# ranrandy/gaussian-splatting-mpm

Hardware: AMD Instinct MI355X
Metric: MPM substeps/sec (and particles·steps/sec) + rendered fps, lego 128³ grid (higher is better)
Workload: dtype f32; 1 GPU; lego.json frame: 100 substeps + postprocess + render 800x800 SH3; particles_per_gpu=100000, particles_total=100000, n_grid=128, material=jelly, render_overlap=True, render_first=False, render_thread=True, render_async=False, parallelism=single

## Files before the change

### gaussian-splatting-mpm_amd/csrc/fused.h

```cpp

#ifndef GSMPM_FT2
#define GSMPM_FT2 7
#endif
constexpr int kFT0 = 8, kFT1 = 8, kFT2 = GSMPM_FT2;
constexpr int kFW0 = kFT0 + 4, kFW1 = kFT1 + 4, kFW2 = kFT2 + 4;
constexpr int kFWin = kFW0 * kFW1 * kFW2;
constexpr int kFTN = kFT0 * kFT1 * kFT2;

__device__ __forceinline__ int slot_loc(int w0, int w1, int w2) { return (w0 * kFW1 + w1) * kFW2 + w2; }

struct SlabWin {
  int W;
  int a[2];
  int on[2];
  float4* part[2];
  int y0[2], ny[2];
  int z0[2], nz[2];
  int* oob;
  int pass;
};

__device__ __forceinline__ int slab_window_of(const SlabWin& sw, int i) {
  if (sw.on[0] && i >= sw.a[0] && i < sw.a[0] + sw.W) return 0;
  if (sw.on[1] && i >= sw.a[1] && i < sw.a[1] + sw.W) return 1;
// ... 15 lines not shown
  int td0, td1, td2;
  int ntiles;
  int max_chunks;
};

struct BinOutF {
  int* count;
  int* ptile;
  int* pslot;
  int* tflag;
  FTiles tl;
};

struct FusedRare {
  BinOutF bo;
  float4* gacc;
  int* esc;
  int* drift;
  int* nonfin;
  const void* bct;
  int* tflag;
  int* touched;
  int* nchunk;
  int4* chunk;
  int2* rcov;
  int* tbox;
  const int* tpos;
  int* rbox;
  const float4* slots_prev;
  const int* tbox_prev;
  const float4* gacc_prev;
  const int* esc_prev;
  const int* esc_old;
  float4* gacc_old;
  int* esc_clr;
  float grav[3];
  unsigned* esc_count;
  float4* esc_nodes;
  unsigned* vmax;
};

constexpr int kFT[3] = {kFT0, kFT1, kFT2};
#ifndef GSMPM_FOLD_BATCH
#define GSMPM_FOLD_BATCH 1
#endif
constexpr int kFoldB = GSMPM_FOLD_BATCH;
__device__ __forceinline__ void fold_axis(int w, int T, int& d, int& sec) {
// ... 136 lines not shown
  tc[0] = b[0] / kFT0;
  tc[1] = b[1] / kFT1;
  tc[2] = b[2] / kFT2;
  return ok ? (tc[0] * tl.td1 + tc[1]) * tl.td2 + tc[2] : tl.ntiles;
}

__device__ __noinline__ void mark8(int* __restrict__ tflag, int t, int td0, int td1, int td2) {
  const int tz = t % td2, ty = (t / td2) % td1, tx = t / (td1 * td2);
  for (int a = 0; a <= 1; ++a)
    for (int b = 0; b <= 1; ++b)
      for (int c = 0; c <= 1; ++c)
        if (tx + a < td0 && ty + b < td1 && tz + c < td2) tflag[((tx + a) * td1 + ty + b) * td2 + tz + c] = 1;
}
__device__ __forceinline__ int reserve_f(const BinOutF& bo, int t, int c) {
  const int old = atomicAdd(&bo.count[t], c);
  if (old == 0 && t < bo.tl.ntiles) mark8(bo.tflag, t, bo.tl.td0, bo.tl.td1, bo.tl.td2);
  return old;
}

struct Touch {
  int* tflag;
  int* touched;
  int* nchunk;
  int4* chunk;
  int* cbox;
  int* tbox;
  unsigned char* perm;
  int2* rcov;
  const int* tpos;
  int* rbox;
};

__device__ __forceinline__ int balanced_lane(const int* __restrict__ rcnt, int cnt, int r, int rank) {
  const int Lr = (cnt - r + 15) >> 4;
  if (rank < Lr) return rank * 16 + r;
  int o = rank - Lr;
  for (int q = 0; q < r; ++q) o += max(0, rcnt[q] - ((cnt - q + 15) >> 4));
  int acc = 0;
  for (int q = 0; q < 16; ++q) {
    const int Lq = (cnt - q + 15) >> 4, d = max(0, Lq - rcnt[q]);
    if (o < acc + d) return (rcnt[q] + (o - acc)) * 16 + q;
    acc += d;
  }
  return rank * 16 + r;
}

constexpr int kFullBox = 0 | (0 << 4) | (0 << 8) | ((kFW0 - 1) << 12) | ((kFW1 - 1) << 16) | ((kFW2 - 1) << 20);
__device__ __forceinline__ void box_unpack(int b, int (&lo)[3], int (&hi)[3]) {
// ... 385 lines not shown
```

### gaussian-splatting-mpm_amd/csrc/fused_body.inc

```
#ifndef GSMPM_FUSED_BODY_INCLUDER
#error "fused_body.inc is the body of k_fused / k_fused_mixed: it is included inside those two kernels in fused.h only"
#endif
  constexpr bool G2P = (MODE & 1) != 0, P2G = (MODE & 2) != 0;
  constexpr bool FOLD = G2P && (MODE & 4) != 0;
  __shared__ int s_fc0[27], s_fnc[27], s_fbx[27];
  constexpr int kEscMax = kFWin / 27;
  __shared__ int s_nesc;
  __shared__ int s_eb[3][kEscMax];
  GridStep fgs{};
  bool fesc = false;
  if constexpr (FOLD) {
    fgs.dt = dt;
    fgs.dgx = dt * rare->grav[0];
    fgs.dgy = dt * rare->grav[1];
    fgs.dgz = dt * rare->grav[2];
    fgs.mask = mask_prev;
    fgs.keep = 0;
    fesc = __builtin_amdgcn_readfirstlane(*rare->esc_prev) != 0;
  }
  __shared__ unsigned long long s_acc[4 * kFWin];
  __shared__ float s_max[4];
  __shared__ int s_mxy[4], s_mz[4];
  __shared__ int s_cnt[27], s_base[27];
  __shared__ int s_rcnt[16];
  float4* s_win = reinterpret_cast<float4*>(s_acc);
  const int ng = g.ng;
  constexpr int SK = (MODE & 3) == 3 ? 0 : 1;
  sim_prio();
  stamp(SK, 0);
  const int w0 = min((int)blockIdx.x, tl.max_chunks - 1);
  const bool perm0 = use_box && tc.perm;
  const int* nch_p = ck.nchunk;
  const int4* chk_p = ck.chunk;
  const int* cbx_p = tc.cbox;
  const unsigned char* prm_p = perm0 ? tc.perm : reinterpret_cast<const unsigned char*>(tc.cbox);
  asm volatile("" : "+s"(nch_p), "+s"(chk_p), "+s"(cbx_p), "+s"(prm_p));
  typedef const int __attribute__((address_space(1)))* gint_p;
  typedef const unsigned char __attribute__((address_space(1)))* guc_p;
  const gint_p c4 = (gint_p)chk_p + 4 * (size_t)w0;
  const int r0 = c4[0], r1 = c4[1], r2 = c4[2], r3 = c4[3];
  const int bx0 = ((gint_p)cbx_p)[w0];
  const int qv0 = ((guc_p)prm_p)[perm0 ? (size_t)w0 * 256 + threadIdx.x : 0];
  const int nch = *(gint_p)nch_p;
  int4 cr_n = make_int4(r0, r1, r2, r3);
  int box_n = use_box ? bx0 : kFullBox;
  int q_n = perm0 ? qv0 : (int)threadIdx.x;
  for (int w = blockIdx.x; w < nch; w += gridDim.x) {
    const int4 cr = cr_n;
    const int cbox = box_n, q_lane = q_n;
    if (w + (int)gridDim.x < nch) {
      const int wn = w + gridDim.x;
      cr_n = ck.chunk[wn];
      box_n = use_box ? tc.cbox[wn] : kFullBox;
      q_n = (use_box && tc.perm) ? (int)tc.perm[(size_t)wn * 256 + threadIdx.x] : (int)threadIdx.x;
    }
    const int t = cr.x, first = cr.y, cnt = cr.z;
    const int k = threadIdx.x;
    const bool outside = t == tl.ntiles;
    int tx = 0, ty = 0, tz = 0;
    if (!outside) ftile_decode(tl, t, tx, ty, tz);
    const int o0 = tx * kFT0 - 1, o1 = ty * kFT1 - 1, o2 = tz * kFT2 - 1;
    int tpos_e = -1;
    const int* __restrict__ tposp = rare->tpos;
    if (tposp && !outside && k < 27) {
      const int x0 = tx - (k / 9 - 1), y0 = ty - ((k / 3) % 3 - 1), z0 = tz - (k % 3 - 1);
      if ((unsigned)x0 < (unsigned)tl.td0 && (unsigned)y0 < (unsigned)tl.td1 && (unsigned)z0 < (unsigned)tl.td2)
        tpos_e = tposp[(x0 * tl.td1 + y0) * tl.td2 + z0];
    }
    int p = -1;
    float x[3] = {0.f, 0.f, 0.f}, v[3] = {0.f, 0.f, 0.f}, C[3][3], F[3][3], m = 0.f;
    const int q = k >= cnt ? k : q_lane;
    if (k < cnt) {
      p = first + q;
#pragma unroll
      for (int d = 0; d < 3; ++d) x[d] = ps.ld(PX + d, p);
      if (G2P || MAT != 0) {
#pragma unroll
        for (int i = 0; i < 9; ++i) F[i / 3][i % 3] = ps.ld(PF + i, p);
      }
      if (P2G) m = ps.ld(PMASS, p);
      if (!G2P) {
#pragma unroll
        for (int d = 0; d < 3; ++d) v[d] = ps.ld(PV + d, p);
#pragma unroll
        for (int i = 0; i < 9; ++i) C[i / 3][i % 3] = ps.ld(PC + i, p);
      }
    }
    int eslot = -1;
    if constexpr (G2P) {
      if (FOLD && !outside) {
        if (k < 27) {
          const int x0 = tx + k / 9 - 1, y0 = ty + (k / 3) % 3 - 1, z0 = tz + k % 3 - 1;
          int c0 = 0, nc = 0, bx = 0;
          if ((unsigned)x0 < (unsigned)tl.td0 && (unsigned)y0 < (unsigned)tl.td1 && (unsigned)z0 < (unsigned)tl.td2) {
            const int u = (x0 * tl.td1 + y0) * tl.td2 + z0;
            c0 = ck.cbase[u];
            nc = (ck.count[u] + kChunk - 1) / kChunk;
            bx = rare->tbox_prev[u];
          }
          s_fc0[k] = c0;
          s_fnc[k] = nc;
          s_fbx[k] = bx;
        }
        if (k == 0) s_nesc = 0;
        __syncthreads();
        if (k < cnt) {
          int bq[3];
          base_of(x, g.inv_dx, bq);
          if (!(in_grid(x, g) && in_window(bq, o0, o1, o2))) {
// ... 37 lines not shown
          }
          float4 vv[kFoldB][8];
#pragma unroll
          for (int u = 0; u < kFoldB; ++u) fold_load(sp, fn[u], vv[u]);
#pragma unroll
          for (int u = 0; u < kFoldB; ++u) {
            const int ix = o0 + w3[u][0], iy = o1 + w3[u][1], iz = o2 + w3[u][2];
            float4 val = make_float4(0.f, 0.f, 0.f, 0.f);
            if (gin[u]) {
              float4 sum = fold_acc(sp, w3[u], tab, fn[u], vv[u]);
              if (fesc) add4f(sum, rare->gacc_prev[((size_t)ix * ng + iy) * ng + iz]);
              val = node_update(sum, ix, iy, iz, g, fgs, fbct);
            }
            if (live[u]) s_win[(w3[u][0] * kFW1 + w3[u][1]) * kFW2 + w3[u][2]] = val;
          }
        }
        __syncthreads();
        const int ne = min(s_nesc, kEscMax);
        for (int t = k; t < ne * 27; t += 256) {
          const int sl = t / 27, qn = t - sl * 27;
          s_win[kFWin + t] = fold_node(s_eb[0][sl] + qn / 9, s_eb[1][sl] + (qn / 3) % 3, s_eb[2][sl] + qn % 3, g, tl,
                                       ck, rare, fgs, fbct, fesc);
        }
      } else if (!outside) {
        int lo[3], hi[3];
        box_unpack(cbox, lo, hi);
        const int n1 = hi[1] - lo[1] + 1, n2 = hi[2] - lo[2] + 1, n12 = n1 * n2;
        const int nvol = (hi[0] - lo[0] + 1) * n12;
        const float r12 = 1.0f / (float)n12, r2 = 1.0f / (float)n2;
        constexpr int kStageU = (kFWin + 255) / 256;
        float4 gv[kStageU];
        int dst[kStageU];
        bool gin[kStageU];
#pragma unroll
        for (int u = 0; u < kStageU; ++u) {
          const int qn = min(k + u * 256, nvol - 1);
          const int a = (int)(((float)qn + 0.5f) * r12), rem = qn - a * n12;
          const int b = (int)(((float)rem + 0.5f) * r2), c = rem - b * n2;
          const int wa = lo[0] + a, wb = lo[1] + b, wc = lo[2] + c;
          dst[u] = (wa * kFW1 + wb) * kFW2 + wc;
          const int ix = o0 + wa, iy = o1 + wb, iz = o2 + wc;
          gin[u] = (unsigned)ix < (unsigned)ng && (unsigned)iy < (unsigned)ng && (unsigned)iz < (unsigned)ng;
          gv[u] = gvel[gin[u] ? ((size_t)ix * ng + iy) * ng + iz : 0];
        }
#pragma unroll
        for (int u = 0; u < kStageU; ++u) {
          const float4 z = gv[u];
          const bool in = gin[u];
          const float4 val = make_float4(in ? z.x : 0.f, in ? z.y : 0.f, in ? z.z : 0.f, in ? z.w : 0.f);
          if (k + u * 256 < nvol) s_win[dst[u]] = val;
        }
      }
      if (k < 27) s_cnt[k] = 0;
      __syncthreads();
      if (w == (int)blockIdx.x) {
        stamp(SK, 2);
        stamp_val(SK, 5, cnt);
        stamp_val(SK, 6, GSMPM_HWREG(4));
        stamp_val(SK, 7, GSMPM_HWREG(20));
      }
      int code = -1, lslot = 0, nt = -1;
      if (k < cnt) {
        int b[3];
        base_of(x, g.inv_dx, b);
        float gvd[3][3];
        const bool inwin = !outside && in_grid(x, g) && in_window(b, o0, o1, o2);
        const bool eslds = eslot >= 0 && eslot < kEscMax;
        if (FOLD && !inwin && !eslds) {
          float4* en = rare->esc_nodes + (size_t)p * 27;
#pragma unroll 1
          for (int qn = 0; qn < 27; ++qn)
            en[qn] = fold_node(b[0] + qn / 9, b[1] + (qn / 3) % 3, b[2] + qn % 3, g, tl, ck, rare, fgs,
                               static_cast<const BcTable*>(rare->bct), fesc);
// ... 167 lines not shown
        for (int r = 0; r < 3; ++r) {
          vm = fmaxf(vm, fabsf(v[r]));
#pragma unroll
          for (int c = 0; c < 3; ++c) {
            cm = fmaxf(cm, fabsf(C[r][c]));
            sm = fmaxf(sm, fabsf(nvt[r][c]));
          }
        }
        bound = fmaxf(m, m * (vm + 4.5f * g.dx * cm) + dt * 4.5f * g.inv_dx * sm) * 1.01f;
      }
      if (outside) {
        if (k < cnt) {
          p2g_global<MAT>(x, v, C, m, nvt, g, dt, rare->gacc);
          int bq[3];
          base_of(x, g.inv_dx, bq);
          mark_escape_tiles(rare->tflag, rare->touched, rare->nchunk + 1, rare->rcov, tl, ng, bq[0], bq[1], bq[2]);
        }
        if (k == 0 && cnt > 0) {
          *rare->esc = 1;
          atomicAdd(rare->esc_count, (unsigned)cnt);
        }
        if (tc.perm && k < cnt) tc.perm[(size_t)w * 256 + k] = (unsigned char)q;
        __syncthreads();
        continue;
      }
      int b[3];
      base_of(x, g.inv_dx, b);
      const bool win = k < cnt && in_grid(x, g) && in_window(b, o0, o1, o2);
      if (k < cnt && (b[0] < xlo || b[0] >= xhi)) *rare->drift = 1;
      int mxy = win ? (7 << (b[0] - o0)) | (7 << (16 + b[1] - o1)) : 0;
      int mz = win ? 7 << (b[2] - o2) : 0;
      if constexpr (GSMPM_DPP_REDUCE != 0) {
        bound = wave_max_nonneg_dpp(bound);
        mxy = wave_or_dpp(mxy);
        mz = wave_or_dpp(mz);
      } else {
#pragma unroll
        for (int o = 32; o > 0; o >>= 1) {
          bound = fmaxf(bound, __shfl_xor(bound, o));
          mxy |= __shfl_xor(mxy, o);
          mz |= __shfl_xor(mz, o);
        }
      }
      if ((k & 63) == 0) {
        s_max[k >> 6] = bound;
        s_mxy[k >> 6] = mxy;
        s_mz[k >> 6] = mz;
      }
      __syncthreads();
      const int res = win ? (((b[0] - o0) * kFW1 + (b[1] - o1)) * kFW2 + (b[2] - o2)) & 15 : (q & 15);
      const int rrank = (tc.perm && k < cnt) ? atomicAdd(&s_rcnt[res], 1) : 0;
      const float bmax = fmaxf(fmaxf(s_max[0], s_max[1]), fmaxf(s_max[2], s_max[3]));
      const int Mxy = s_mxy[0] | s_mxy[1] | s_mxy[2] | s_mxy[3], Mz = s_mz[0] | s_mz[1] | s_mz[2] | s_mz[3];
      const int Mx = Mxy & 0xffff, My = (unsigned)Mxy >> 16;
      const int lo_all = (Mx & 1) | ((My & 1) << 1) | ((Mz & 1) << 2);
      if (lo_all & ~cr.w) {
        Touch tr = tc;
        tr.tflag = rare->tflag;
        tr.touched = rare->touched;
        tr.nchunk = rare->nchunk;
        tr.rcov = rare->rcov;
        add_lower_tiles(tr, tl, tx, ty, tz, (lo_all | cr.w) & 7);
        if (k == 0) rare->chunk[w].w = lo_all | cr.w;
      }
      int box = kFullBox;
      if (Mx && My && Mz)
        box = (__builtin_ctz(Mx)) | (__builtin_ctz(My) << 4) | (__builtin_ctz(Mz) << 8) | ((31 - __builtin_clz(Mx)) << 12) |
              ((31 - __builtin_clz(My)) << 16) | ((31 - __builtin_clz(Mz)) << 20);
      else
        box = 0;
      if (k == 0) {
        tc.cbox[w] = box;
        rare->tbox[t] = (cr.w & 8) ? kFullBox : box;
      }
      if (tpos_e >= 0) rare->rbox[(size_t)tpos_e * kRecStride + k] = (cr.w & 8) ? kFullBox : box;
      if (cr.w & 8) box = kFullBox;
      int ebits;
      frexpf(bmax, &ebits);
      const int S = bmax > 0.f ? 50 - ebits : 0;
      if (k < cnt) {
        if (win) {
          int bb[3];
          float fx[3], ww[3][3], dw[3][3];
          bspline(x, g.inv_dx, bb, fx, ww, dw);
          p2g_scatter<MAT, kFW1, kFW2, kFWin>(s_acc + ((b[0] - o0) * kFW1 + (b[1] - o1)) * kFW2 + (b[2] - o2), fx, ww,
                                              dw, v, C, m, nvt, g, dt, ldexp(1.0, S));
        } else {
          p2g_global<MAT>(x, v, C, m, nvt, g, dt, rare->gacc);
          *rare->esc = 1;
        }
      }
      {
        const unsigned long long eb = __ballot(k < cnt && !win);
        if (eb) {
          if ((k & 63) == 0) atomicAdd(rare->esc_count, (unsigned)__popcll(eb));
// ... 4 lines not shown
      __syncthreads();
      if (w == (int)blockIdx.x) stamp(SK, 4);
      if (tc.perm && k < cnt) tc.perm[(size_t)w * 256 + balanced_lane(s_rcnt, cnt, res, rrank)] = (unsigned char)q;
      int lo[3], hi[3];
      box_unpack(box, lo, hi);
      const int n1 = hi[1] - lo[1] + 1, n2 = hi[2] - lo[2] + 1, n12 = n1 * n2;
      const int nvol = (hi[0] - lo[0] + 1) * n12;
      const float r12 = 1.0f / (float)n12, r2 = 1.0f / (float)n2;
      const int cid = (cr.w & 16) ? (int)((unsigned)cr.w >> 5) : w;
      float4* dst = slots + (size_t)cid * kFWin;
      for (int qn = k; qn < nvol; qn += 256) {
        const int a = (int)(((float)qn + 0.5f) * r12), rem = qn - a * n12;
        const int bq = (int)(((float)rem + 0.5f) * r2), c = rem - bq * n2;
        const int node = ((lo[0] + a) * kFW1 + lo[1] + bq) * kFW2 + lo[2] + c;
        float4 r;
        r.x = from_fixed32(s_acc[0 * kFWin + node], S);
        r.y = from_fixed32(s_acc[1 * kFWin + node], S);
        r.z = from_fixed32(s_acc[2 * kFWin + node], S);
        r.w = from_fixed32(s_acc[3 * kFWin + node], S);
        wt_store4(dst + node, r);
      }
      __syncthreads();
    }
  }
  if (bin == 2) {
    const BinOutF bo = rare->bo;
    for (int t = blockIdx.x * 256 + threadIdx.x; t <= tl.ntiles; t += gridDim.x * 256) {
      bo.count[t] = 0;
      if (t < tl.ntiles) bo.tflag[t] = 0;
    }
  }
  if (rare->esc_clr) {
    if (__builtin_amdgcn_readfirstlane(*rare->esc_old) != 0) {
      const size_t nn = (size_t)ng * ng * ng;
      for (size_t q = (size_t)blockIdx.x * 256 + threadIdx.x; q < nn; q += (size_t)gridDim.x * 256)
        rare->gacc_old[q] = make_float4(0.f, 0.f, 0.f, 0.f);
    }
    if (blockIdx.x == 0 && threadIdx.x == 0) *rare->esc_clr = 0;
  }
  stamp(SK, 1);
```

### gaussian-splatting-mpm_amd/csrc/mpm.hip

```cpp
#include <hip/hip_runtime.h>
#include <dlfcn.h>


#include <algorithm>
#include <climits>
#include <cmath>
#include <cstring>
#include <map>
#include <numeric>
#include <vector>

#include "common.h"
#include "constitutive.h"
#include <hip/hip_ext.h>

#include "mpm_common.h"
#include "svd3.h"

namespace gsmpm {

#ifndef GSMPM_REBIN_SF
#define GSMPM_REBIN_SF 20
#endif
constexpr int kRebinStressFree = GSMPM_REBIN_SF;
// ... 777 lines not shown
    if (w == (int)blockIdx.x) stamp(1, 4);
    if (p >= 0) {
      bo.ptile[p] = nt;
      bo.pslot[p] = code >= 0 ? s_base[code] + lslot : reserve(bo, nt, 1);
    }
    __syncthreads();
  }
  stamp(1, 1);
}

__global__ __launch_bounds__(256) void k_bin_all(Particles ps, GridDims g, Tiles tl, BinOut bo) {
  const int p = blockIdx.x * blockDim.x + threadIdx.x;
  if (p < ps.n) {
    float x[3];
#pragma unroll
    for (int d = 0; d < 3; ++d) x[d] = ps.ld(PX + d, p);
    int tc[3];
    const int t = tile_of(x, g, tl, tc);
    bo.ptile[p] = t;
    bo.pslot[p] = reserve(bo, t, 1);
  }
}

struct ChunkOut {
  int* cstart;
  int* cbase;
  int4* chunk;
  int* nchunk;
  const int* tflag;
  int* touched;
  int2* rcov = nullptr;
  int* tpos = nullptr;
  int td1 = 0, td2 = 0;
};

constexpr int kRecStride = 32;
__device__ __forceinline__ void write_cover_record(const ChunkOut& co, int ntiles, int E, int t, int rk,
                                                   const int* s_off, const int* s_aux, int total) {
  const int td12 = co.td1 * co.td2, td0 = ntiles / td12;
  const int tz = t % co.td2, ty = (t / co.td2) % co.td1, tx = t / td12;
  for (int e = 0; e < 27; ++e) {
    const int x = tx + e / 9 - 1, y = ty + (e / 3) % 3 - 1, z = tz + e % 3 - 1;
    int2 r = make_int2(0, 0);
    if ((unsigned)x < (unsigned)td0 && (unsigned)y < (unsigned)co.td1 && (unsigned)z < (unsigned)co.td2) {
      const int u = (x * co.td1 + y) * co.td2 + z;
      const int cnt = (u + 1 < E ? s_off[u + 1] : total) - s_off[u];
      r = make_int2(s_aux[u] & 0xffff, (cnt + kChunk - 1) / kChunk);
    }
    co.rcov[(size_t)rk * kRecStride + e] = r;
  }
  co.rcov[(size_t)rk * kRecStride + 27] = make_int2(0, 0);
}

__device__ __forceinline__ int wave_incl_scan(int v) {
  const int lane = threadIdx.x & 63;
#pragma unroll
// ... 69 lines not shown
  for (int t = t0; t < t1; ++t) {
    const int e = s_off[t], c = e & INT_MAX;
    v[0] += c;
    v[1] += (c + kChunk - 1) / kChunk;
    v[2] += e < 0;
  }
  int o[3], tot[3];
  block_scan3(v, o, tot);
  stamp(2, 3);
  for (int t = t0; t < t1; ++t) {
    const int e = s_off[t], c = e & INT_MAX;
    s_off[t] = o[0];
    s_aux[t] = o[1] | (o[2] << 16);
    o[0] += c;
    o[1] += (c + kChunk - 1) / kChunk;
    o[2] += e < 0;
  }
  if (blockIdx.x == 0 && threadIdx.x == 0) {
    co.nchunk[0] = tot[1];
    co.nchunk[1] = tot[2];
  }
  __syncthreads();
  stamp(2, 4);
  const int R = (E + gridDim.x - 1) / gridDim.x;
  for (int t = blockIdx.x * R + threadIdx.x; t < min(E, (int)(blockIdx.x + 1) * R); t += 256) {
    const int off = s_off[t], aux = s_aux[t];
    const int c = (t + 1 < E ? s_off[t + 1] : tot[0]) - off;
    const int cb = aux & 0xffff, rk = aux >> 16;
    const bool touched = (t + 1 < E ? (s_aux[t + 1] >> 16) : tot[2]) > rk;
    co.cbase[t] = cb;
    for (int k = 0; k * kChunk < c; ++k)
      co.chunk[cb + k] = make_int4(t, off + k * kChunk, min(kChunk, c - k * kChunk), c > kChunk ? 8 : 0);
    if (touched) co.touched[rk] = t;
    if (co.tpos && t < tl.ntiles) {
      co.tpos[t] = touched ? rk : -1;
      if (touched) write_cover_record(co, tl.ntiles, E, t, rk, s_off, s_aux, tot[0]);
    }
  }
  if (p < n) {
    const int d = s_off[pt] + psl;
    if (bp.dst) {
      float v[NPLANES];
      const bool skip = bp.skip_vc != 0;
#pragma unroll
      for (int q = 0; q < NPLANES; ++q)
        if (!(skip && q >= PV && q < PF)) v[q] = bp.src[(size_t)q * bp.np + p];
      const int o = bp.osrc[p];
#pragma unroll
      for (int q = 0; q < NPLANES; ++q)
        if (!(skip && q >= PV && q < PF)) bp.dst[(size_t)q * bp.np + d] = v[q];
      bp.odst[d] = o;
    } else {
      list[d] = p;
    }
  }
// ... 55 lines not shown
  tile_values(tl, count, co.tflag, t, v);
  int inc[3];
#pragma unroll
  for (int r = 0; r < 3; ++r) {
    inc[r] = wave_incl_scan(v[r]);
    if (lane == 63) s_wsum[r][wave] = inc[r];
  }
  __syncthreads();
  if (threadIdx.x < 64) {
#pragma unroll
    for (int r = 0; r < 3; ++r) {
      const int x = lane < 16 ? s_wsum[r][lane] : 0;
      const int xi = wave_incl_scan(x);
      if (lane < 16) s_wsum[r][lane] = xi - x;
    }
  }
  __syncthreads();
  int o[3];
#pragma unroll
  for (int r = 0; r < 3; ++r) o[r] = carry[r] + s_wsum[r][wave] + inc[r] - v[r];
  if (t < E) {
    co.cstart[t] = o[0];
    co.cbase[t] = o[1];
    for (int k = 0; k < v[1]; ++k)
      co.chunk[o[1] + k] = make_int4(t, o[0] + k * kChunk, min(kChunk, v[0] - k * kChunk), v[0] > kChunk ? 8 : 0);
    if (v[2]) co.touched[o[2]] = t;
    if (co.tpos && t < tl.ntiles) co.tpos[t] = -1;
    if (v[2] && co.rcov) co.rcov[(size_t)o[2] * kRecStride + 27] = make_int2(1, 0);
  }
  if (blockIdx.x == gridDim.x - 1 && threadIdx.x == 1023) {
    co.nchunk[0] = o[1] + v[1];
    co.nchunk[1] = o[2] + v[2];
  }
}

__global__ __launch_bounds__(256) void k_scatter(int n, const int* __restrict__ nlive, const int* __restrict__ ptile,
                                                 const int* __restrict__ pslot, const int* __restrict__ cstart,
                                                 int* __restrict__ list) {
  const int p = blockIdx.x * blockDim.x + threadIdx.x;
  if (p >= (nlive ? *nlive : n)) return;
  list[cstart[ptile[p]] + pslot[p]] = p;
}


#include "fused.h"
#include "slab.h"
#include "lsd.h"

__global__ __launch_bounds__(256) void k_postprocess(Particles ps, const int* __restrict__ orig) {
  const int p = blockIdx.x * blockDim.x + threadIdx.x;
  if (p >= ps.n) return;
  const int o = orig[p];
  float F[3][3];
#pragma unroll
  for (int i = 0; i < 9; ++i) F[i / 3][i % 3] = ps.ld(PF + i, p);
// ... 322 lines not shown
struct MemRec {
  void* p;
  size_t bytes;
  MemGroup group;
};

struct BinLists {
  int* count = nullptr;
  int* cstart = nullptr;
  int* cbase = nullptr;
  int4* chunk = nullptr;
  int* nchunk = nullptr;
  int* touched = nullptr;
  int* tflag = nullptr;
  int* list = nullptr;
};
struct PhasedBufs {
  float4* slots = nullptr;
  BinLists b[2];
};
struct FusedBufs {
  float4* slots = nullptr;
  BinLists b[2];
  int* cbox[2] = {nullptr, nullptr};
  int* tbox[2] = {nullptr, nullptr};
  int2* rcov[2] = {nullptr, nullptr};
  int* rbox[2] = {nullptr, nullptr};
  int* tpos[2] = {nullptr, nullptr};
  unsigned char* perm[2] = {nullptr, nullptr};
  int4* pchunk[2] = {nullptr, nullptr};
  float* planes_alt = nullptr;
  int* orig_alt = nullptr;
  int* esc = nullptr;
  FusedRare* rare_dev = nullptr;
  unsigned* vmax_dev = nullptr;
  float* vmax_host = nullptr;
};
struct FoldBufs {
  float4* slots2 = nullptr;
  float4* gacc[2] = {nullptr, nullptr};
  int* tbox2[2] = {nullptr, nullptr};
  float4* esc_nodes = nullptr;
};

struct gsmpm_mpm {
  gsmpm_mpm_params prm{};
  GridDims g{};
  MatConsts mc{};
  Tiles tl{};
  int mat_kernel = 0;
  float* mat_ids = nullptr;
  bool mixed = false;
  bool rebin_set = false;
// ... 156 lines not shown
static const int* nlive_of(const gsmpm_mpm* h) { return h->slab ? h->d_n : nullptr; }

static ChunkIn chunk_in(const BinLists& b, int4* records) {
  return ChunkIn{b.count, b.cbase, records, b.nchunk, b.list, b.touched};
}
static ChunkOut chunk_out(const BinLists& b) {
  return ChunkOut{b.cstart, b.cbase, b.chunk, b.nchunk, b.tflag, b.touched};
}

static ChunkIn chunk_in(gsmpm_mpm* h, int c) { return chunk_in(h->ph.b[c], h->ph.b[c].chunk); }
static ChunkOut chunk_out(gsmpm_mpm* h, int c) { return chunk_out(h->ph.b[c]); }
static BinOut bin_out(gsmpm_mpm* h, int c) {
  return BinOut{h->ph.b[c].count, h->ptile, h->pslot, h->ph.b[c].tflag, h->tl.td, h->tl.ntiles};
}

static bool use_fused(const gsmpm_mpm* h) { return h->fused; }
static const BinLists& bin_lists(const gsmpm_mpm* h, int c) { return use_fused(h) ? h->fu.b[c] : h->ph.b[c]; }

static int kernel_code(const gsmpm_mpm* h) { return h->mixed ? kMatMixed : h->mat_kernel; }
static MatIds<kMatMixed> mat_ids_of(gsmpm_mpm* h) {
  return MatIds<kMatMixed>{h->mat_ids, h->orig, (h->prm.flags & GSMPM_FLAG_JELLY_FCR) ? 4 : 0};
}

static int4* fused_records(gsmpm_mpm* h, int c) {
  return h->chunk_order ? h->fu.pchunk[c] : h->fu.b[c].chunk;
}
static ChunkIn chunk_in_f(gsmpm_mpm* h, int c) {
  ChunkIn ci = chunk_in(h->fu.b[c], fused_records(h, c));
  if (h->cover_records) {
    ci.rcov = h->fu.rcov[c];
    ci.rbox = h->fu.rbox[c];
  }
  return ci;
}
static ChunkOut chunk_out_f(gsmpm_mpm* h, int c) {
  ChunkOut co = chunk_out(h->fu.b[c]);
  co.rcov = h->fu.rcov[c];
  co.tpos = h->fu.tpos[c];
  co.td1 = h->ftl.td1;
  co.td2 = h->ftl.td2;
  return co;
}
static Touch touch_f(gsmpm_mpm* h, int c) {
  const BinLists& b = h->fu.b[c];
  return Touch{b.tflag, b.touched, b.nchunk, b.chunk, h->fu.cbox[c], h->fu.tbox[c],
               h->lane_balance ? h->fu.perm[c] : nullptr, h->fu.rcov[c],
               h->cover_records ? h->fu.tpos[c] : nullptr, h->fu.rbox[c]};
}
static BinOutF bin_out_f(gsmpm_mpm* h, int c) {
  return BinOutF{h->fu.b[c].count, h->ptile, h->pslot, h->fu.b[c].tflag, h->ftl};
}
static Tiles ftiles_flat(const gsmpm_mpm* h) { return Tiles{h->ftl.td0, h->ftl.ntiles, h->ftl.max_chunks}; }

static int p2g_grid(gsmpm_mpm* h) { return std::min(h->tl.max_chunks, 1024); }
static int g2p_grid(gsmpm_mpm* h) { return std::min(h->tl.max_chunks, 1024); }
static int grid_grid(gsmpm_mpm* h) { return std::min(h->tl.ntiles, 1024); }

template <typename F, typename... Args>
static void launch(const hipEvent_t* ev, F kernel, dim3 grid, dim3 block, hipStream_t st, Args... args) {
  if (ev)
    hipExtLaunchKernelGGL(kernel, grid, block, 0, st, ev[0], ev[1], 0, args...);
  else
    hipLaunchKernelGGL(kernel, grid, block, 0, st, args...);
}

template <int MAT>
static void launch_p2g(gsmpm_mpm* h, int c, uint32_t mask, float dt, hipStream_t st, const hipEvent_t* ev) {
  if constexpr (MAT == kMatMixed)
// ... 5 lines not shown
}

static bool bins_fused(const Tiles& tl) { return tl.ntiles + 1 <= kFuseTiles && tl.max_chunks < 65536; }
static int finish_bins_on(gsmpm_mpm* h, const Tiles& tl, const int* count, const ChunkOut& co, int* list,
                          hipStream_t st, const hipEvent_t* ev, const BinPermute& bp = BinPermute{}) {
  if (bins_fused(tl)) {
    launch(ev, k_finish_bins, dim3(std::max(1, div_up(live_rows(h), 256))), dim3(256), st, tl, count, co, h->n,
           nlive_of(h), (const int*)h->ptile, (const int*)h->pslot, list, bp);
  } else {
    const hipEvent_t e0[2] = {ev ? ev[0] : nullptr, nullptr}, e1[2] = {nullptr, ev ? ev[1] : nullptr};
    const int nblk = div_up(tl.ntiles + 1, 1024);
    launch(ev ? e0 : nullptr, k_scan_partials, dim3(nblk), dim3(1024), st, tl, count, (const int*)co.tflag,
           h->scan_part);
    launch(nullptr, k_scan_tiles, dim3(nblk), dim3(1024), st, tl, count, co, (const int4*)h->scan_part);
    launch(ev ? e1 : nullptr, k_scatter, dim3(std::max(1, div_up(live_rows(h), 256))), dim3(256), st, h->n,
           nlive_of(h), (const int*)h->ptile, (const int*)h->pslot, (const int*)co.cstart, list);
  }
  GSMPM_LAUNCH_CHECK();
  return GSMPM_OK;
}
static int finish_binning(gsmpm_mpm* h, int c, hipStream_t st, const hipEvent_t* ev = nullptr) {
  return finish_bins_on(h, h->tl, h->ph.b[c].count, chunk_out(h, c), h->ph.b[c].list, st, ev);
}
__device__ __forceinline__ void order_by_size(const int4* __restrict__ chunk, int nch, int4* __restrict__ pchunk,
                                              int ncu) {
  __shared__ int s_h[kChunk];
  for (int i = threadIdx.x; i < kChunk; i += blockDim.x) s_h[i] = 0;
  __syncthreads();
  for (int c = threadIdx.x; c < nch; c += blockDim.x) atomicAdd(&s_h[kChunk - chunk[c].z], 1);
  __syncthreads();
  if (threadIdx.x < 64) {
    int v[kChunk / 64], t = 0;
#pragma unroll
    for (int u = 0; u < kChunk / 64; ++u) {
      v[u] = s_h[threadIdx.x * (kChunk / 64) + u];
      t += v[u];
    }
    int o = wave_incl_scan(t) - t;
#pragma unroll
    for (int u = 0; u < kChunk / 64; ++u) {
      s_h[threadIdx.x * (kChunk / 64) + u] = o;
      o += v[u];
    }
  }
  __syncthreads();
  const int full = nch / ncu;
  for (int c = threadIdx.x; c < nch; c += blockDim.x) {
    const int4 r = chunk[c];
    const int rank = atomicAdd(&s_h[kChunk - r.z], 1);
    const int tier = rank / ncu, i = rank - tier * ncu;
    const int pos = tier * ncu + (((tier & 1) && tier < full) ? ncu - 1 - i : i);
    pchunk[pos] = make_int4(r.x, r.y, r.z, r.w | 16 | (c << 5));
  }
}
__global__ __launch_bounds__(1024) void k_chunk_order(const int4* __restrict__ chunk, const int* __restrict__ nchunk,
                                                      int4* __restrict__ pchunk, int ncu) {
  order_by_size(chunk, *nchunk, pchunk, ncu);
}
constexpr int kOrdMax = 4096;
__global__ __launch_bounds__(1024) void k_chunk_order_xcd(const int4* __restrict__ chunk, const int* __restrict__ nchunk,
                                                          const int* __restrict__ tpos, int ntiles,
                                                          int4* __restrict__ pchunk, int ncu) {
  __shared__ int s_h[8][kChunk];
  __shared__ unsigned char s_x[kOrdMax];
  __shared__ unsigned short s_r[kOrdMax];
  __shared__ int s_n[8], s_cap[8], s_def[9], s_ovf;
  const int nch = *nchunk;
  if (nch > kOrdMax) {
    order_by_size(chunk, nch, pchunk, ncu);
    return;
  }
  for (int i = threadIdx.x; i < 8 * kChunk; i += blockDim.x) (&s_h[0][0])[i] = 0;
  if (threadIdx.x < 8) s_n[threadIdx.x] = 0;
  if (threadIdx.x == 0) s_ovf = 0;
  __syncthreads();
  const int T = (nch + 7) / 8, rem = nch - 8 * (T - 1);
  for (int c = threadIdx.x; c < nch; c += blockDim.x) {
    const int t = chunk[c].x;
    const int P = t < ntiles ? tpos[t] : -1;
    const int x = P >= 0 ? (P / kGridGroup) & 7 : c & 7;
    s_x[c] = (unsigned char)x;
    s_r[c] = (unsigned short)atomicAdd(&s_n[x], 1);
  }
  __syncthreads();
  if (threadIdx.x == 0) {
    int d = 0;
    for (int x = 0; x < 8; ++x) {
      s_cap[x] = x < rem ? T : T - 1;
      s_def[x] = d;
      d += max(0, s_cap[x] - s_n[x]);
    }
    s_def[8] = d;
  }
  __syncthreads();
// ... 11 lines not shown
  if (threadIdx.x < 8 * 64) {
    const int x = threadIdx.x >> 6, l = threadIdx.x & 63;
    int v[kChunk / 64], t = 0;
#pragma unroll
    for (int u = 0; u < kChunk / 64; ++u) {
      v[u] = s_h[x][l * (kChunk / 64) + u];
      t += v[u];
    }
    int o = wave_incl_scan(t) - t;
#pragma unroll
    for (int u = 0; u < kChunk / 64; ++u) {
      s_h[x][l * (kChunk / 64) + u] = o;
      o += v[u];
    }
  }
  __syncthreads();
  const int cpx = max(1, ncu / 8);
  for (int c = threadIdx.x; c < nch; c += blockDim.x) {
    const int4 r = chunk[c];
    const int x = s_x[c];
    const int rank = atomicAdd(&s_h[x][kChunk - r.z], 1);
    const int tier = rank / cpx, i = rank - tier * cpx, full = s_cap[x] / cpx;
    const int j = tier * cpx + (((tier & 1) && tier < full) ? cpx - 1 - i : i);
    pchunk[j * 8 + x] = make_int4(r.x, r.y, r.z, r.w | 16 | (c << 5));
  }
}
#ifndef GSMPM_CHUNK_XCD
#define GSMPM_CHUNK_XCD 1
#endif
static int order_chunks_f(gsmpm_mpm* h, int c, hipStream_t st) {
  if (!h->chunk_order) return GSMPM_OK;
  if (GSMPM_CHUNK_XCD && kGridGroup > 0 && std::min(h->ftl.max_chunks, h->fused_wgs) % 8 == 0)
    launch(nullptr, k_chunk_order_xcd, dim3(1), dim3(1024), st, (const int4*)h->fu.b[c].chunk,
           (const int*)h->fu.b[c].nchunk, (const int*)h->fu.tpos[c], h->ftl.ntiles, h->fu.pchunk[c], h->ncu);
  else
    launch(nullptr, k_chunk_order, dim3(1), dim3(1024), st, (const int4*)h->fu.b[c].chunk,
           (const int*)h->fu.b[c].nchunk, h->fu.pchunk[c], h->ncu);
  GSMPM_LAUNCH_CHECK();
  return GSMPM_OK;
}
static int finish_binning_f(gsmpm_mpm* h, int c, hipStream_t st, const hipEvent_t* ev = nullptr) {
  const int rc = finish_bins_on(h, ftiles_flat(h), h->fu.b[c].count, chunk_out_f(h, c), h->fu.b[c].list, st, ev);
  return rc ? rc : order_chunks_f(h, c, st);
}
static int permute_to_bins(gsmpm_mpm* h, int c, hipStream_t st, const hipEvent_t* ev);
static int rebin_permute_f(gsmpm_mpm* h, int c, hipStream_t st, const hipEvent_t* ev = nullptr, bool vc_live = true) {
  if (bins_fused(ftiles_flat(h)) && h->fuse_permute) {
    const BinPermute bp{h->planes, h->fu.planes_alt, h->np,
                        h->orig,   h->fu.orig_alt,   (vc_live || GSMPM_STORE_VC) ? 0 : 1};
    int rc = finish_bins_on(h, ftiles_flat(h), h->fu.b[c].count, chunk_out_f(h, c), h->fu.b[c].list, st, ev, bp);
    if (!rc) rc = order_chunks_f(h, c, st);
    if (rc) return rc;
    if (ev) {
      GSMPM_HIP(hipEventRecord(ev[2], st));
      GSMPM_HIP(hipEventRecord(ev[3], st));
    }
    std::swap(h->planes, h->fu.planes_alt);
    std::swap(h->orig, h->fu.orig_alt);
    return GSMPM_OK;
  }
// ... 115 lines not shown
constexpr int kFoldPhases = 12;
static float4* fold_slots(gsmpm_mpm* h, int r) { return (r & 1) ? h->fo.slots2 : h->fu.slots; }
static int* fold_tbox(gsmpm_mpm* h, int c, int r) { return (r & 1) ? h->fo.tbox2[c] : h->fu.tbox[c]; }
static int* fold_flag(gsmpm_mpm* h, int r) { return h->fu.esc + 2 + ((r % kFoldPhases) + kFoldPhases) % kFoldPhases; }
static float4* fold_gacc(gsmpm_mpm* h, int r) {
  const int i = ((r % 3) + 3) % 3;
  return i ? h->fo.gacc[i - 1] : h->gacc;
}
static int* fold_scratch(gsmpm_mpm* h) { return h->fu.esc + 2 + kFoldPhases; }

static FusedRare rare_of(gsmpm_mpm* h, int c, int slot) {
  FusedRare r{};
  const bool fold = slot >= 2;
  const int ph = slot - 2;
  r.bo = bin_out_f(h, c ^ 1);
  r.gacc = fold ? fold_gacc(h, ph) : h->gacc;
  r.esc = fold ? fold_flag(h, ph) : h->fu.esc + slot;
  r.drift = h->slab ? h->s_drift : nullptr;
  r.nonfin = h->slab ? h->s_drift + SF_NONFIN : h->nonfin_dev;
  r.bct = h->dev_bc;
  r.tflag = h->fu.b[c].tflag;
  r.touched = h->fu.b[c].touched;
  r.nchunk = h->fu.b[c].nchunk;
  r.chunk = fused_records(h, c);
  r.rcov = h->fu.rcov[c];
  r.tbox = fold ? fold_tbox(h, c, ph) : h->fu.tbox[c];
  r.tpos = h->cover_records ? h->fu.tpos[c] : nullptr;
  r.rbox = h->fu.rbox[c];
  if (fold) {
    r.slots_prev = fold_slots(h, ph + 1);
    r.tbox_prev = fold_tbox(h, c, ph + 1);
    r.gacc_prev = fold_gacc(h, ph - 1);
    r.esc_prev = fold_flag(h, ph - 1);
    r.esc_old = fold_flag(h, ph - 2);
    r.gacc_old = fold_gacc(h, ph - 2);
    r.esc_clr = fold_flag(h, ph - 3);
  }
  for (int d = 0; d < 3; ++d) r.grav[d] = (float)h->prm.gravity[d];
  r.esc_count = reinterpret_cast<unsigned*>(h->fu.esc + 3 + kFoldPhases);
  r.esc_nodes = h->fo.esc_nodes;
  r.vmax = h->slab ? nullptr : h->fu.vmax_dev;
  return r;
}
static int sync_rare(gsmpm_mpm* h, hipStream_t st) {
  bool dirty = false;
  for (int i = 0; i < 2 * kRareSlots; ++i) {
    if (i % kRareSlots >= 2 && !h->fold) continue;
// ... 505 lines not shown
    if (const char* fw = std::getenv("GSMPM_FUSED_WGS")) h->fused_wgs = std::max(1, std::atoi(fw));
    if (const char* co = std::getenv("GSMPM_CHUNK_ORDER")) h->chunk_order = co[0] != '0';
  }
  h->ftl.td0 = (h->g.ng + kFT0 - 1) / kFT0;
  h->ftl.td1 = (h->g.ng + kFT1 - 1) / kFT1;
  h->ftl.td2 = (h->g.ng + kFT2 - 1) / kFT2;
  h->ftl.ntiles = h->ftl.td0 * h->ftl.td1 * h->ftl.td2;
  h->ftl.max_chunks = h->n / kChunk + std::min(h->ftl.ntiles + 1, h->n) + 1;
  if (h->fused && sizeof(float4) * (size_t)(h->ftl.max_chunks + 1) * kFWin > 0xffffffffull) h->fused = false;
  if (const char* fo = std::getenv("GSMPM_FOLD")) h->fold = h->fused && fo[0] != '0';
  if (const char* ra = std::getenv("GSMPM_REBIN_AUTO")) h->rebin_auto = h->fused && ra[0] != '0';
  if (!h->fused) {
    GSMPM_TRY(alloc(h, &h->ph.slots, (size_t)(h->tl.max_chunks + 1) * kWin, kMemPhased, kFillZero,
                    (size_t)h->tl.max_chunks * kWin),
              "chunk slots");
    for (BinLists& b : h->ph.b)
      GSMPM_TRY(alloc_bin_lists(h, b, h->tl.ntiles, h->tl.max_chunks, kMemPhased), "bin lists");
  } else {
    FusedBufs& f = h->fu;
    const size_t nt = (size_t)h->ftl.ntiles, mc = (size_t)h->ftl.max_chunks;
    GSMPM_TRY(alloc(h, &f.slots, (mc + 1) * kFWin, kMemFused, kFillZero, mc * kFWin), "fused slots");
    for (int c = 0; c < 2; ++c) {
      GSMPM_TRY(alloc_bin_lists(h, f.b[c], h->ftl.ntiles, h->ftl.max_chunks, kMemFused), "bin lists");
      GSMPM_TRY(alloc(h, &f.cbox[c], mc, kMemFused), "boxes");
      GSMPM_TRY(alloc(h, &f.pchunk[c], mc, kMemFused, kFillZero), "ordered chunks");
      GSMPM_TRY(alloc(h, &f.tbox[c], nt, kMemFused), "boxes");
      GSMPM_TRY(alloc(h, &f.rcov[c], kRecStride * nt, kMemFused, kFillZero), "cover records");
      GSMPM_TRY(alloc(h, &f.rbox[c], kRecStride * nt, kMemFused, kFillZero), "cover boxes");
      GSMPM_TRY(alloc(h, &f.tpos[c], nt, kMemFused, kFillOnes), "touched positions");
      GSMPM_TRY(alloc(h, &f.perm[c], mc * 256, kMemFused, kFillZero), "lane balance");
    }
    GSMPM_TRY(alloc(h, &f.planes_alt, (size_t)NPLANES * h->np, kMemFused, kFillZero), "planes");
    GSMPM_TRY(alloc(h, &f.orig_alt, (size_t)h->np, kMemFused), "orig");
    GSMPM_TRY(alloc(h, &f.esc, 4 + kFoldPhases, kMemFused, kFillZero), "escape flags");
    GSMPM_TRY(alloc(h, &f.vmax_dev, 1, kMemFused, kFillZero), "vmax");
    GSMPM_TRY(alloc_host(h, &f.vmax_host, 1), "pinned vmax");
    *f.vmax_host = 0.f;
    GSMPM_TRY(alloc(h, &f.rare_dev, 2 * kRareSlots, kMemFused, kFillZero), "rare args");
    if (h->fold) {
      GSMPM_TRY(alloc(h, &h->fo.slots2, (mc + 1) * kFWin, kMemFold, kFillZero, mc * kFWin), "fused slots");
      for (float4*& g : h->fo.gacc) GSMPM_TRY(alloc(h, &g, nn, kMemFold, kFillZero), "grid acc");
      GSMPM_TRY(alloc(h, &h->fo.esc_nodes, 27 * (size_t)h->np, kMemFold), "escape nodes");
      for (int*& t : h->fo.tbox2) GSMPM_TRY(alloc(h, &t, nt, kMemFold, kFillZero), "boxes");
    }
  }
  const int scan_tiles = std::max(h->tl.ntiles, h->ftl.ntiles) + 1;
  GSMPM_TRY(alloc(h, &h->scan_part, (size_t)div_up(scan_tiles, 1024), kMemCommon), "scan partials");
  GSMPM_TRY(alloc(h, &h->ptile, (size_t)h->np, kMemCommon), "ptile");
// ... 740 lines not shown
```

Baseline: 3.293 billion particle-substeps/s.

## Pack chunk record and box into launch records and prefetch next chunk earlier

Merges the per-chunk int4 record and the box word into one 32-byte LaunchRec, so the fused kernel fetches the next chunk's metadata with a single vector load plus one int. Unused trailing records are cleared to a sentinel, which lets the loop stop on that marker and converts the loaded fields to scalar registers via readfirstlane. The prefetch of the next record is issued earlier, right after the particle loads or the grid staging, and consumed at the end of the iteration, to hide the load latency of the serial chunk loop. The change adds clearing work in the binning and ordering kernels and reworks loop control, which could introduce bugs when records are stale.

Result: no change. 3.272 billion particle-substeps/s (-0.6%).

```diff
diff --git a/gaussian-splatting-mpm_amd/csrc/fused.h b/gaussian-splatting-mpm_amd/csrc/fused.h
--- a/gaussian-splatting-mpm_amd/csrc/fused.h
+++ b/gaussian-splatting-mpm_amd/csrc/fused.h
@@ -61,7 +61,7 @@
   int* tflag;
   int* touched;
   int* nchunk;
-  int4* chunk;
+  LaunchRec* lrec;
   int2* rcov;
   int* tbox;
   const int* tpos;
@@ -244,8 +244,7 @@
   int* tflag;
   int* touched;
   int* nchunk;
-  int4* chunk;
-  int* cbox;
+  LaunchRec* lrec;
   int* tbox;
   unsigned char* perm;
   int2* rcov;
diff --git a/gaussian-splatting-mpm_amd/csrc/fused_body.inc b/gaussian-splatting-mpm_amd/csrc/fused_body.inc
--- a/gaussian-splatting-mpm_amd/csrc/fused_body.inc
+++ b/gaussian-splatting-mpm_amd/csrc/fused_body.inc
@@ -28,32 +28,44 @@
   constexpr int SK = (MODE & 3) == 3 ? 0 : 1;
   sim_prio();
   stamp(SK, 0);
-  const int w0 = min((int)blockIdx.x, tl.max_chunks - 1);
   const bool perm0 = use_box && tc.perm;
+  const LaunchRec* lr_p = tc.lrec;
   const int* nch_p = ck.nchunk;
-  const int4* chk_p = ck.chunk;
-  const int* cbx_p = tc.cbox;
-  const unsigned char* prm_p = perm0 ? tc.perm : reinterpret_cast<const unsigned char*>(tc.cbox);
-  asm volatile("" : "+s"(nch_p), "+s"(chk_p), "+s"(cbx_p), "+s"(prm_p));
+  const unsigned char* prm_p = perm0 ? tc.perm : reinterpret_cast<const unsigned char*>(tc.lrec);
+  asm volatile("" : "+s"(lr_p), "+s"(nch_p), "+s"(prm_p));
+  typedef int i4v __attribute__((ext_vector_type(4)));
+  typedef const i4v __attribute__((address_space(1)))* gi4_p;
   typedef const int __attribute__((address_space(1)))* gint_p;
   typedef const unsigned char __attribute__((address_space(1)))* guc_p;
-  const gint_p c4 = (gint_p)chk_p + 4 * (size_t)w0;
-  const int r0 = c4[0], r1 = c4[1], r2 = c4[2], r3 = c4[3];
-  const int bx0 = ((gint_p)cbx_p)[w0];
-  const int qv0 = ((guc_p)prm_p)[perm0 ? (size_t)w0 * 256 + threadIdx.x : 0];
-  const int nch = *(gint_p)nch_p;
-  int4 cr_n = make_int4(r0, r1, r2, r3);
-  int box_n = use_box ? bx0 : kFullBox;
-  int q_n = perm0 ? qv0 : (int)threadIdx.x;
-  for (int w = blockIdx.x; w < nch; w += gridDim.x) {
+  i4v ra = *(gi4_p)(lr_p + blockIdx.x);
+  int rb = ((gint_p)(lr_p + blockIdx.x))[4];
+  int rq = ((guc_p)prm_p)[perm0 ? (size_t)blockIdx.x * 256 + threadIdx.x : 0];
+  int rn = *(gint_p)nch_p;
+  asm volatile("" : "+v"(ra), "+v"(rb), "+v"(rq), "+v"(rn));
+  const int nch = __builtin_amdgcn_readfirstlane(rn);
+  int4 cr_n = make_int4(__builtin_amdgcn_readfirstlane(ra.x), __builtin_amdgcn_readfirstlane(ra.y),
+                        __builtin_amdgcn_readfirstlane(ra.z), __builtin_amdgcn_readfirstlane(ra.w));
+  int box_n = use_box ? __builtin_amdgcn_readfirstlane(rb) : kFullBox;
+  int q_n = perm0 ? rq : (int)threadIdx.x;
+  bool go = cr_n.x != kNoChunk;
+  for (int w = blockIdx.x; go; w += gridDim.x) {
     const int4 cr = cr_n;
     const int cbox = box_n, q_lane = q_n;
-    if (w + (int)gridDim.x < nch) {
-      const int wn = w + gridDim.x;
-      cr_n = ck.chunk[wn];
-      box_n = use_box ? tc.cbox[wn] : kFullBox;
-      q_n = (use_box && tc.perm) ? (int)tc.perm[(size_t)wn * 256 + threadIdx.x] : (int)threadIdx.x;
-    }
+    const bool more = w + (int)gridDim.x < nch;
+    int wl = more ? w + (int)gridDim.x : w;
+    asm volatile("" : "+s"(wl));
+    auto request_next = [&]() {
+      ra = *(gi4_p)(lr_p + wl);
+      rb = ((gint_p)(lr_p + wl))[4];
+      rq = ((guc_p)prm_p)[perm0 ? (size_t)wl * 256 + threadIdx.x : 0];
+    };
+    auto take_next = [&]() {
+      asm volatile("" : "+v"(ra), "+v"(rb), "+v"(rq));
+      cr_n = make_int4(__builtin_amdgcn_readfirstlane(ra.x), __builtin_amdgcn_readfirstlane(ra.y),
+                       __builtin_amdgcn_readfirstlane(ra.z), __builtin_amdgcn_readfirstlane(ra.w));
+      box_n = use_box ? __builtin_amdgcn_readfirstlane(rb) : kFullBox;
+      q_n = perm0 ? rq : (int)threadIdx.x;
+    };
     const int t = cr.x, first = cr.y, cnt = cr.z;
     const int k = threadIdx.x;
     const bool outside = t == tl.ntiles;
@@ -85,6 +97,9 @@
 #pragma unroll
         for (int i = 0; i < 9; ++i) C[i / 3][i % 3] = ps.ld(PC + i, p);
       }
+    }
+    if constexpr (!G2P || FOLD) {
+      if (more) request_next();
     }
     int eslot = -1;
     if constexpr (G2P) {
@@ -168,7 +183,7 @@
           s_win[kFWin + t] = fold_node(s_eb[0][sl] + qn / 9, s_eb[1][sl] + (qn / 3) % 3, s_eb[2][sl] + qn % 3, g, tl,
                                        ck, rare, fgs, fbct, fesc);
         }
-      } else if (!outside) {
+      } else if constexpr (!FOLD) {
         int lo[3], hi[3];
         box_unpack(cbox, lo, hi);
         const int n1 = hi[1] - lo[1] + 1, n2 = hi[2] - lo[2] + 1, n12 = n1 * n2;
@@ -189,12 +204,14 @@
           gin[u] = (unsigned)ix < (unsigned)ng && (unsigned)iy < (unsigned)ng && (unsigned)iz < (unsigned)ng;
           gv[u] = gvel[gin[u] ? ((size_t)ix * ng + iy) * ng + iz : 0];
         }
+        if (more) request_next();
+        const int nst = outside ? 0 : nvol;
 #pragma unroll
         for (int u = 0; u < kStageU; ++u) {
           const float4 z = gv[u];
           const bool in = gin[u];
           const float4 val = make_float4(in ? z.x : 0.f, in ? z.y : 0.f, in ? z.z : 0.f, in ? z.w : 0.f);
-          if (k + u * 256 < nvol) s_win[dst[u]] = val;
+          if (k + u * 256 < nst) s_win[dst[u]] = val;
         }
       }
       if (k < 27) s_cnt[k] = 0;
@@ -408,6 +425,8 @@
         }
         if (tc.perm && k < cnt) tc.perm[(size_t)w * 256 + k] = (unsigned char)q;
         __syncthreads();
+        if (more) take_next();
+        go = more;
         continue;
       }
       int b[3];
@@ -447,7 +466,7 @@
         tr.nchunk = rare->nchunk;
         tr.rcov = rare->rcov;
         add_lower_tiles(tr, tl, tx, ty, tz, (lo_all | cr.w) & 7);
-        if (k == 0) rare->chunk[w].w = lo_all | cr.w;
+        if (k == 0) rare->lrec[w].rec.w = lo_all | cr.w;
       }
       int box = kFullBox;
       if (Mx && My && Mz)
@@ -456,7 +475,7 @@
       else
         box = 0;
       if (k == 0) {
-        tc.cbox[w] = box;
+        tc.lrec[w].box = box;
         rare->tbox[t] = (cr.w & 8) ? kFullBox : box;
       }
       if (tpos_e >= 0) rare->rbox[(size_t)tpos_e * kRecStride + k] = (cr.w & 8) ? kFullBox : box;
@@ -507,6 +526,8 @@
       }
       __syncthreads();
     }
+    if (more) take_next();
+    go = more;
   }
   if (bin == 2) {
     const BinOutF bo = rare->bo;
diff --git a/gaussian-splatting-mpm_amd/csrc/mpm.hip b/gaussian-splatting-mpm_amd/csrc/mpm.hip
--- a/gaussian-splatting-mpm_amd/csrc/mpm.hip
+++ b/gaussian-splatting-mpm_amd/csrc/mpm.hip
@@ -823,6 +823,16 @@
   }
 }
 
+constexpr int kNoChunk = -1;
+struct alignas(32) LaunchRec {
+  int4 rec;
+  int box;
+  int pad[3];
+};
+__device__ __forceinline__ void clear_launch_recs(LaunchRec* __restrict__ lrec, int from, int to, int lane, int lanes) {
+  for (int i = from + lane; i < to; i += lanes) lrec[i].rec = make_int4(kNoChunk, 0, 0, 0);
+}
+
 struct ChunkOut {
   int* cstart;
   int* cbase;
@@ -833,6 +843,8 @@
   int2* rcov = nullptr;
   int* tpos = nullptr;
   int td1 = 0, td2 = 0;
+  LaunchRec* lrec = nullptr;
+  int lgrid = 0;
 };
 
 constexpr int kRecStride = 32;
@@ -948,6 +960,7 @@
   }
   __syncthreads();
   stamp(2, 4);
+  if (co.lrec) clear_launch_recs(co.lrec, tot[1], co.lgrid, blockIdx.x * 256 + threadIdx.x, gridDim.x * 256);
   const int R = (E + gridDim.x - 1) / gridDim.x;
   for (int t = blockIdx.x * R + threadIdx.x; t < min(E, (int)(blockIdx.x + 1) * R); t += 256) {
     const int off = s_off[t], aux = s_aux[t];
@@ -955,8 +968,11 @@
     const int cb = aux & 0xffff, rk = aux >> 16;
     const bool touched = (t + 1 < E ? (s_aux[t + 1] >> 16) : tot[2]) > rk;
     co.cbase[t] = cb;
-    for (int k = 0; k * kChunk < c; ++k)
-      co.chunk[cb + k] = make_int4(t, off + k * kChunk, min(kChunk, c - k * kChunk), c > kChunk ? 8 : 0);
+    for (int k = 0; k * kChunk < c; ++k) {
+      const int4 r = make_int4(t, off + k * kChunk, min(kChunk, c - k * kChunk), c > kChunk ? 8 : 0);
+      co.chunk[cb + k] = r;
+      if (co.lrec) co.lrec[cb + k].rec = r;
+    }
     if (touched) co.touched[rk] = t;
     if (co.tpos && t < tl.ntiles) {
       co.tpos[t] = touched ? rk : -1;
@@ -1058,8 +1074,11 @@
   if (t < E) {
     co.cstart[t] = o[0];
     co.cbase[t] = o[1];
-    for (int k = 0; k < v[1]; ++k)
-      co.chunk[o[1] + k] = make_int4(t, o[0] + k * kChunk, min(kChunk, v[0] - k * kChunk), v[0] > kChunk ? 8 : 0);
+    for (int k = 0; k < v[1]; ++k) {
+      const int4 r = make_int4(t, o[0] + k * kChunk, min(kChunk, v[0] - k * kChunk), v[0] > kChunk ? 8 : 0);
+      co.chunk[o[1] + k] = r;
+      if (co.lrec) co.lrec[o[1] + k].rec = r;
+    }
     if (v[2]) co.touched[o[2]] = t;
     if (co.tpos && t < tl.ntiles) co.tpos[t] = -1;
     if (v[2] && co.rcov) co.rcov[(size_t)o[2] * kRecStride + 27] = make_int2(1, 0);
@@ -1067,6 +1086,12 @@
   if (blockIdx.x == gridDim.x - 1 && threadIdx.x == 1023) {
     co.nchunk[0] = o[1] + v[1];
     co.nchunk[1] = o[2] + v[2];
+  }
+  if (co.lrec && blockIdx.x == gridDim.x - 1) {
+    __shared__ int s_nch;
+    if (threadIdx.x == 1023) s_nch = o[1] + v[1];
+    __syncthreads();
+    clear_launch_recs(co.lrec, s_nch, co.lgrid, threadIdx.x, 1024);
   }
 }
 
@@ -1435,13 +1460,12 @@
 struct FusedBufs {
   float4* slots = nullptr;
   BinLists b[2];
-  int* cbox[2] = {nullptr, nullptr};
   int* tbox[2] = {nullptr, nullptr};
   int2* rcov[2] = {nullptr, nullptr};
   int* rbox[2] = {nullptr, nullptr};
   int* tpos[2] = {nullptr, nullptr};
   unsigned char* perm[2] = {nullptr, nullptr};
-  int4* pchunk[2] = {nullptr, nullptr};
+  LaunchRec* lrec[2] = {nullptr, nullptr};
   float* planes_alt = nullptr;
   int* orig_alt = nullptr;
   int* esc = nullptr;
@@ -1644,11 +1668,8 @@
   return MatIds<kMatMixed>{h->mat_ids, h->orig, (h->prm.flags & GSMPM_FLAG_JELLY_FCR) ? 4 : 0};
 }
 
-static int4* fused_records(gsmpm_mpm* h, int c) {
-  return h->chunk_order ? h->fu.pchunk[c] : h->fu.b[c].chunk;
-}
 static ChunkIn chunk_in_f(gsmpm_mpm* h, int c) {
-  ChunkIn ci = chunk_in(h->fu.b[c], fused_records(h, c));
+  ChunkIn ci = chunk_in(h->fu.b[c], h->fu.b[c].chunk);
   if (h->cover_records) {
     ci.rcov = h->fu.rcov[c];
     ci.rbox = h->fu.rbox[c];
@@ -1661,11 +1682,15 @@
   co.tpos = h->fu.tpos[c];
   co.td1 = h->ftl.td1;
   co.td2 = h->ftl.td2;
+  if (!h->chunk_order) {
+    co.lrec = h->fu.lrec[c];
+    co.lgrid = std::min(h->ftl.max_chunks, h->fused_wgs);
+  }
   return co;
 }
 static Touch touch_f(gsmpm_mpm* h, int c) {
   const BinLists& b = h->fu.b[c];
-  return Touch{b.tflag, b.touched, b.nchunk, b.chunk, h->fu.cbox[c], h->fu.tbox[c],
+  return Touch{b.tflag, b.touched, b.nchunk, h->fu.lrec[c], h->fu.tbox[c],
                h->lane_balance ? h->fu.perm[c] : nullptr, h->fu.rcov[c],
                h->cover_records ? h->fu.tpos[c] : nullptr, h->fu.rbox[c]};
 }
@@ -1717,8 +1742,9 @@
 static int finish_binning(gsmpm_mpm* h, int c, hipStream_t st, const hipEvent_t* ev = nullptr) {
   return finish_bins_on(h, h->tl, h->ph.b[c].count, chunk_out(h, c), h->ph.b[c].list, st, ev);
 }
-__device__ __forceinline__ void order_by_size(const int4* __restrict__ chunk, int nch, int4* __restrict__ pchunk,
-                                              int ncu) {
+__device__ __forceinline__ void order_by_size(const int4* __restrict__ chunk, int nch, LaunchRec* __restrict__ lrec,
+                                              int lgrid, int ncu) {
+  clear_launch_recs(lrec, nch, lgrid, threadIdx.x, blockDim.x);
   __shared__ int s_h[kChunk];
   for (int i = threadIdx.x; i < kChunk; i += blockDim.x) s_h[i] = 0;
   __syncthreads();
@@ -1745,26 +1771,27 @@
     const int rank = atomicAdd(&s_h[kChunk - r.z], 1);
     const int tier = rank / ncu, i = rank - tier * ncu;
     const int pos = tier * ncu + (((tier & 1) && tier < full) ? ncu - 1 - i : i);
-    pchunk[pos] = make_int4(r.x, r.y, r.z, r.w | 16 | (c << 5));
+    lrec[pos].rec = make_int4(r.x, r.y, r.z, r.w | 16 | (c << 5));
   }
 }
 __global__ __launch_bounds__(1024) void k_chunk_order(const int4* __restrict__ chunk, const int* __restrict__ nchunk,
-                                                      int4* __restrict__ pchunk, int ncu) {
-  order_by_size(chunk, *nchunk, pchunk, ncu);
+                                                      LaunchRec* __restrict__ lrec, int lgrid, int ncu) {
+  order_by_size(chunk, *nchunk, lrec, lgrid, ncu);
 }
 constexpr int kOrdMax = 4096;
 __global__ __launch_bounds__(1024) void k_chunk_order_xcd(const int4* __restrict__ chunk, const int* __restrict__ nchunk,
                                                           const int* __restrict__ tpos, int ntiles,
-                                                          int4* __restrict__ pchunk, int ncu) {
+                                                          LaunchRec* __restrict__ lrec, int lgrid, int ncu) {
   __shared__ int s_h[8][kChunk];
   __shared__ unsigned char s_x[kOrdMax];
   __shared__ unsigned short s_r[kOrdMax];
   __shared__ int s_n[8], s_cap[8], s_def[9], s_ovf;
   const int nch = *nchunk;
   if (nch > kOrdMax) {
-    order_by_size(chunk, nch, pchunk, ncu);
+    order_by_size(chunk, nch, lrec, lgrid, ncu);
     return;
   }
+  clear_launch_recs(lrec, nch, lgrid, threadIdx.x, blockDim.x);
   for (int i = threadIdx.x; i < 8 * kChunk; i += blockDim.x) (&s_h[0][0])[i] = 0;
   if (threadIdx.x < 8) s_n[threadIdx.x] = 0;
   if (threadIdx.x == 0) s_ovf = 0;
@@ -1822,7 +1849,7 @@
     const int rank = atomicAdd(&s_h[x][kChunk - r.z], 1);
     const int tier = rank / cpx, i = rank - tier * cpx, full = s_cap[x] / cpx;
     const int j = tier * cpx + (((tier & 1) && tier < full) ? cpx - 1 - i : i);
-    pchunk[j * 8 + x] = make_int4(r.x, r.y, r.z, r.w | 16 | (c << 5));
+    lrec[j * 8 + x].rec = make_int4(r.x, r.y, r.z, r.w | 16 | (c << 5));
   }
 }
 #ifndef GSMPM_CHUNK_XCD
@@ -1830,12 +1857,13 @@
 #endif
 static int order_chunks_f(gsmpm_mpm* h, int c, hipStream_t st) {
   if (!h->chunk_order) return GSMPM_OK;
-  if (GSMPM_CHUNK_XCD && kGridGroup > 0 && std::min(h->ftl.max_chunks, h->fused_wgs) % 8 == 0)
+  const int lgrid = std::min(h->ftl.max_chunks, h->fused_wgs);
+  if (GSMPM_CHUNK_XCD && kGridGroup > 0 && lgrid % 8 == 0)
     launch(nullptr, k_chunk_order_xcd, dim3(1), dim3(1024), st, (const int4*)h->fu.b[c].chunk,
-           (const int*)h->fu.b[c].nchunk, (const int*)h->fu.tpos[c], h->ftl.ntiles, h->fu.pchunk[c], h->ncu);
+           (const int*)h->fu.b[c].nchunk, (const int*)h->fu.tpos[c], h->ftl.ntiles, h->fu.lrec[c], lgrid, h->ncu);
   else
     launch(nullptr, k_chunk_order, dim3(1), dim3(1024), st, (const int4*)h->fu.b[c].chunk,
-           (const int*)h->fu.b[c].nchunk, h->fu.pchunk[c], h->ncu);
+           (const int*)h->fu.b[c].nchunk, h->fu.lrec[c], lgrid, h->ncu);
   GSMPM_LAUNCH_CHECK();
   return GSMPM_OK;
 }
@@ -1997,7 +2025,7 @@
   r.tflag = h->fu.b[c].tflag;
   r.touched = h->fu.b[c].touched;
   r.nchunk = h->fu.b[c].nchunk;
-  r.chunk = fused_records(h, c);
+  r.lrec = h->fu.lrec[c];
   r.rcov = h->fu.rcov[c];
   r.tbox = fold ? fold_tbox(h, c, ph) : h->fu.tbox[c];
   r.tpos = h->cover_records ? h->fu.tpos[c] : nullptr;
@@ -2549,8 +2577,7 @@
     GSMPM_TRY(alloc(h, &f.slots, (mc + 1) * kFWin, kMemFused, kFillZero, mc * kFWin), "fused slots");
     for (int c = 0; c < 2; ++c) {
       GSMPM_TRY(alloc_bin_lists(h, f.b[c], h->ftl.ntiles, h->ftl.max_chunks, kMemFused), "bin lists");
-      GSMPM_TRY(alloc(h, &f.cbox[c], mc, kMemFused), "boxes");
-      GSMPM_TRY(alloc(h, &f.pchunk[c], mc, kMemFused, kFillZero), "ordered chunks");
+      GSMPM_TRY(alloc(h, &f.lrec[c], mc, kMemFused, kFillZero), "launch records");
       GSMPM_TRY(alloc(h, &f.tbox[c], nt, kMemFused), "boxes");
       GSMPM_TRY(alloc(h, &f.rcov[c], kRecStride * nt, kMemFused, kFillZero), "cover records");
       GSMPM_TRY(alloc(h, &f.rbox[c], kRecStride * nt, kMemFused, kFillZero), "cover boxes");
```
